# Samaretas/global-motion-estimation

Hardware: AMD Instinct MI355X
Metric: frame-pairs/s + achieved HBM GB/s, 720x480 bs=16 sw=16 exhaustive (higher is better)
Workload: dtype u8; 1 GPU; 720x480 synthetic luma, bs=16 sw=16 exhaustive MAE (BASELINE configs[1]); frame_distance=1, streams_per_gpu=1, collective=none, exchange=none in this run, multi_gpu_measured_by_builder=False

## Files before the change

global-motion-estimation_amd/csrc/bbme_sea.hip:

```cpp
#include "bbme_sea_common.h"

namespace {

using namespace sea;

constexpr int GUARD_NONE = 0, GUARD_ROWS = 1, GUARD_ALL = 2;
constexpr uint32_t PENALTY = 1u << 17;
constexpr uint32_t FIRST_INVALID_KEY = 65536u << 13;
constexpr uint32_t FIRST_INVALID_BOUND = FIRST_INVALID_KEY >> 13;
__device__ __forceinline__ uint32_t lds_add_rtn(uint32_t* p, uint32_t v)
{
    uint32_t old;
    const uint32_t addr = (uint32_t)(uintptr_t)(__attribute__((address_space(3))) uint32_t*)p;
    asm volatile("ds_add_rtn_u32 %0, %1, %2\n\ts_waitcnt lgkmcnt(0)" : "=v"(old) : "v"(addr), "v"(v) : "memory");
    return old;
}
constexpr uint32_t ENT_INTERIOR = 1u << 29;
__device__ __forceinline__ int wave_row(const SeaGeo& d, int w)
{
    if (__builtin_constant_p(d.tc) && (d.tc & (d.tc - 1)) == 0) return w >> __builtin_ctz((unsigned)d.tc);
    return div_small(w, d.magic_tc);
}
__device__ __forceinline__ uint64_t any_u64()
{
// ... 132 lines not shown
            for (int s = 0; s < 4; ++s) w[s] = *(const u64_a4*)(lrow + t * d.pitch_dw + s);
#pragma unroll
            for (int i = 0; i < R; ++i) {
                const int a = t - i;
                if (a < 0 || a > 3) continue;
                const u32x4 ar = *(const u32x4*)(an + a * 4);
#pragma unroll
                for (int j = 0; j < 4; ++j)
                    acc[i] = __builtin_amdgcn_qsad_pk_u16_u8(w[j], ar[j], acc[i]);
            }
        }
    }
#pragma unroll
    for (int i = 0; i < R; ++i) {
        uint32_t lo = (uint32_t)acc[i], hi = (uint32_t)(acc[i] >> 32);
        lo += (uint32_t)__builtin_amdgcn_update_dpp(0, (int)lo, 0xB1, 0xF, 0xF, false);
        hi += (uint32_t)__builtin_amdgcn_update_dpp(0, (int)hi, 0xB1, 0xF, 0xF, false);
        lo += (uint32_t)__builtin_amdgcn_update_dpp(0, (int)lo, 0x4E, 0xF, 0xF, false);
        hi += (uint32_t)__builtin_amdgcn_update_dpp(0, (int)hi, 0x4E, 0xF, 0xF, false);
        asm volatile("" : "+v"(lo), "+v"(hi));
        acc[i] = ((uint64_t)hi << 32) | lo;
    }
    uint32_t key = 0xFFFFFFFFu;
    if (active) {
        const int ci = q2 * 4 * R + 4 * k2 + sub, ri0 = prow2 * R;
        const uint32_t shift = (uint32_t)(sub & 1) * 16u;
        if (ent & ENT_INTERIOR) {
#pragma unroll
            for (int i = 0; i < R; ++i) {
                const uint32_t word = (sub & 2) ? (uint32_t)(acc[i] >> 32) : (uint32_t)acc[i];
                const uint32_t sad = __builtin_amdgcn_ubfe(word, shift, 16u);
                key = min(key, (sad << 13) + (uint32_t)i);
            }
            key += (uint32_t)(ci * NC + ri0);
        } else {
            const int c02 = (bcol0 + wc2) * 16, r02 = (trow * d.tr + wr2) * 16;
            const int lo_c = max(0, d.sw - c02), hi_c = min(NC - 1, W - 16 - c02 + d.sw);
            const int lo_r2 = max(0, d.sw - r02), hi_r2 = min(NC - 1, H - 16 - r02 + d.sw);
#pragma unroll
            for (int i = 0; i < R; ++i) {
                const int ri = ri0 + i;
                if (ci < lo_c || ci > hi_c || ri < lo_r2 || ri > hi_r2) continue;
                const uint32_t word = (sub & 2) ? (uint32_t)(acc[i] >> 32) : (uint32_t)acc[i];
                const uint32_t sad = __builtin_amdgcn_ubfe(word, shift, 16u);
                key = min(key, (sad << 13) | (uint32_t)(ci * NC + ri));
            }
        }
        key = min(key, (uint32_t)__builtin_amdgcn_update_dpp(-1, (int)key, 0xB1, 0xF, 0xF, false));
        key = min(key, (uint32_t)__builtin_amdgcn_update_dpp(-1, (int)key, 0x4E, 0xF, 0xF, false));
    }
    return key;
}

template <int R, bool FIXED, bool VERT>
__device__ __forceinline__ bool tile_phases(const SeaGeo& d, uint32_t* lds, const Layout& L, int pair, int trow, int bcol0,
                                            uint32_t mine, uint32_t pa, uint32_t pb, int tid, int tile_id, PhaseClock& clk)
{
    constexpr bool E4 = R >= 3;
    const int T = blockDim.x;
    const int NC = 2 * d.sw + 16, XQ = d.xq;
    uint32_t* win = lds + L.win;
    uint32_t* anchor = lds + L.anchor;
    uint32_t* best = lds + L.best;
    uint32_t* count = lds + L.count;
    uint64_t* s8 = (uint64_t*)(lds + L.s8);
    uint32_t* work = lds + L.work;
    const int wave = __builtin_amdgcn_readfirstlane(tid >> 6);
    const int lane = tid & 63;
    const SeaArgs c = launch_args();
    const WaveBlock wb = wave_block(d, c, trow, bcol0, wave);
    const int brow = wb.brow, bcol = wb.bcol;
    const bool wave_ok = wb.ok;
    const int r0 = brow * 16, c0 = bcol * 16;
    const int prow = lane >> 2, q = lane & 3;

    box_sums8<R, FIXED>(d, win, s8, tid);
    clk.mark(ST_BOX, lane);
    __syncthreads();
    clk.mark(ST_BOX_WAIT, lane);

    const int lo_r = max(0, d.sw - r0), hi_r = min(NC - 1, c->H - 16 - r0 + d.sw);
    const bool rows_inside = NC == 16 * R && lo_r == 0 && hi_r == NC - 1;
    uint32_t ub_key = 0xFFFFFFFFu;
    if (wave_ok) {
        const int lo_c = max(0, d.sw - c0), hi_c = min(NC - 1, c->W - 16 - c0 + d.sw);
        uint32_t pmin[R];
        const uint64_t* s8blk = s8 + 16 * wb.wr * XQ + wb.wc * 4;
        const uint64_t* sp0 = s8blk + prow * R * XQ + q * R;
        const bool cols_inside = NC == 16 * R && lo_c == 0 && hi_c == NC - 1;
        if (rows_inside && cols_inside)
            lower_bounds<R, GUARD_NONE, VERT>(sp0, XQ, prow, q, pa, pb, lo_r, hi_r, lo_c, hi_c, pmin);
        else if (R <= 3 && cols_inside)
            lower_bounds<R, GUARD_ROWS, VERT>(sp0, XQ, prow, q, pa, pb, lo_r, hi_r, lo_c, hi_c, pmin);
        else
            lower_bounds<R, GUARD_ALL, VERT>(sp0, XQ, prow, q, pa, pb, lo_r, hi_r, lo_c, hi_c, pmin);
        const uint32_t first_idx = (uint32_t)((q * 4 * R) * NC + prow * R);
        const uint32_t ent0 = (rows_inside && cols_inside ? ENT_INTERIOR : 0u) | ((uint32_t)wave << 25) | ((uint32_t)lane << 19);
        uint32_t pkd[R], lane_min = 0xFFFFFFFFu;
#pragma unroll
        for (int k = 0; k < R; ++k) {
            pkd[k] = (pmin[k] << 13) | (first_idx + (uint32_t)(4 * k * NC));
            lane_min = min(lane_min, pmin[k]);
        }
        const uint32_t lane_lb = lane_min << 13;
        uint32_t lb_key = lane_min != 0xFFFFFFFFu ? lane_lb + ((uint32_t)lane << 7) : 0xFFFFFFFFu;
        lb_key = wave_min_u32(lb_key);
        {
            const int idx1 = min_bound_candidate<R, VERT>(s8blk, XQ, NC, (int)(lb_key >> 7) & 63, lb_key >> 13, pa, pb,
                                                          lo_r, hi_r, lo_c, hi_c, lane);
            const int idx0 = d.sw * NC + d.sw;
            const int arow = lane >> 2, aj = lane & 3;
            uint32_t packed = 0;
#pragma unroll
            for (int which = 0; which < 2; ++which) {
                const int idx = which ? idx1 : idx0;
                const int ci = idx / NC, ri = idx - ci * NC;
                const int byte = wb.wc * 16 + ci + 4 * aj;
                const uint32_t* p = win + (16 * wb.wr + ri + arow) * d.pitch_dw + (byte >> 2);
                const uint32_t v = __builtin_amdgcn_alignbyte(p[1], p[0], (uint32_t)byte & 3u);
                packed += __builtin_amdgcn_sad_u8(v, mine, 0u) << (16 * which);
            }
            packed = wave_sum_u32(packed);
            ub_key = min(((packed & 0xFFFFu) << 13) | (uint32_t)idx0, ((packed >> 16) << 13) | (uint32_t)idx1);
            const int idxp = (int)(best[2 * wave + 1] & 0x1FFFu);
            const int cip = idxp / NC, rip = idxp - cip * NC;
            if (idxp != idx0 && idxp != idx1 && cip >= lo_c && cip <= hi_c && rip >= lo_r && rip <= hi_r) {
                const int byte = wb.wc * 16 + cip + 4 * aj;
                const uint32_t* p = win + (16 * wb.wr + rip + arow) * d.pitch_dw + (byte >> 2);
                const uint32_t v = __builtin_amdgcn_alignbyte(p[1], p[0], (uint32_t)byte & 3u);
                const uint32_t sadp = wave_sum_u32(__builtin_amdgcn_sad_u8(v, mine, 0u));
                ub_key = min(ub_key, (sadp << 13) | (uint32_t)idxp);
            }
// ... 200 lines not shown
                        }
                    key += (uint32_t)(ci0 * NC + ri0);
                } else {
                    const int c02 = (bcol0 + wc2) * 16, r02 = (trow * d.tr + wr2) * 16;
                    const int lo_c = max(0, d.sw - c02), hi_c = min(NC - 1, W - 16 - c02 + d.sw);
                    const int lo_r2 = max(0, d.sw - r02), hi_r2 = min(NC - 1, H - 16 - r02 + d.sw);
    #pragma unroll
                    for (int e4 = 0; e4 < 4; ++e4) {
                        const int ci = ci0 + e4;
                        if (ci < lo_c || ci > hi_c) continue;
    #pragma unroll
                        for (int i = 0; i < R; ++i) {
                            const int ri = ri0 + i;
                            if (ri < lo_r2 || ri > hi_r2) continue;
                            const uint32_t sad = (uint32_t)(acc[i] >> (16 * e4)) & 0xFFFFu;
                            key = min(key, (sad << 13) | (uint32_t)(ci * NC + ri));
                        }
                    }
                }
                if (key != 0xFFFFFFFFu) atomicMin(&best[2 * w2], key);
            }
            clk.mark(ST_E, lane);
            __syncthreads();
            clk.mark(ST_E_WAIT, lane);
        }

    }
    if (wave_ok && lane == 0) {
        const int idx = (int)(best[2 * wave] & 0x1FFF);
        const int ci = idx / NC, ri = idx - ci * NC;
        int32_t* o = ce->mf + (((long long)pair * ce->nbr + brow) * ce->nbc + bcol) * 2;
        o[0] = ci - d.sw;
        o[1] = ri - d.sw;
        best[2 * wave + 1] = (uint32_t)idx;
    }
    return false;
}

template <int R, bool FIXED = false, bool VERT = true>
struct MaeTile {
    struct Pre { uint32_t pa, pb; };
    static __device__ __forceinline__ Pre prep(uint32_t* lds, const Layout& L, int wave, int lane, bool wave_ok, uint32_t mine)
    {
        Pre p = { 0, 0 };
        if (wave_ok) {
            lds[L.anchor + wave * ANCHOR_STRIDE + lane] = mine;
            uint32_t a01, a23;
            anchor_quadrants(mine, &a01, &a23);
            p.pa = VERT ? pair_u16(a01, a23, false) : a01;
            p.pb = VERT ? pair_u16(a01, a23, true) : a23;
        }
        return p;
    }
    static __device__ __forceinline__ bool phases(const SeaGeo& d, uint32_t* lds, const Layout& L, int pair, int trow, int bcol0,
                                                  uint32_t mine, const Pre& p, int tid, int tile_id, PhaseClock& clk)
    {
        return tile_phases<R, FIXED, VERT>(d, lds, L, pair, trow, bcol0, mine, p.pa, p.pb, tid, tile_id, clk);
    }
    static __device__ __forceinline__ int probe_word(const Layout& L, int wave) { return L.best + 2 * wave + 1; }
};

template <int R>
__global__ void __launch_bounds__(1024) k_exh_sea16(SeaDev d)
{
    extern __shared__ uint32_t lds[];
    const SeaGeo g = d;
    one_tile<MaeTile<R>>(g, lds, layout_of(g, R));
}

constexpr bool vertical_pairs(int R, int NV) { return !(R == 5 && NV == 16); }

template <int R, int NV, int GEO = 0>
__global__ void __launch_bounds__(1024, (R <= 3 ? 8 : 6)) k_exh_sea16p(SeaDev d)
{
    extern __shared__ uint32_t lds[];
    SeaGeo g = d;
    fix_geometry<R, GEO>(g);
    const Layout L = layout_of(g, R);
    if ((threadIdx.x & 63) == 0) lds[L.best + 2 * (threadIdx.x >> 6) + 1] = (uint32_t)(g.sw * (2 * g.sw + 16) + g.sw);
    persistent_tiles<NV, MaeTile<R, GEO != 0, vertical_pairs(R, NV)>>(g, lds, L);
}

struct MaeLaunch {
    static constexpr const char* persistent_name = "k_exh_sea16p";
    static constexpr const char* one_tile_name = "k_exh_sea16";
    static int no_plan()
    {
        gme_set_error("search window too large for LDS");
        return GME_ERR_ARG;
    }
    static void tables(SeaDev& d, const BbmeJob&) { d.sqbox = nullptr; d.sqbox_stride = 0; }
    static void ordered(SeaDev& d)
    {
        d.quota = getenv("GME_SEA_QUOTA") ? atoi(getenv("GME_SEA_QUOTA")) : SEA_DEFAULT_QUOTA;
        d.bisect = getenv("GME_SEA_BISECT") ? atoi(getenv("GME_SEA_BISECT")) : SEA_DEFAULT_BISECT;
        d.engage = getenv("GME_SEA_ENGAGE") ? atoi(getenv("GME_SEA_ENGAGE")) : SEA_DEFAULT_ENGAGE;
        if (d.engage < d.quota) d.engage = d.quota;
    }
    static bool fits(int R, int nv) { return R <= 1 || R >= 4 || nv <= 8; }
    template <int R, int NV, int GEO = 0>
    static void persistent(dim3 grid, dim3 block, size_t lds, hipStream_t s, const SeaDev& d)
    {
        hipLaunchKernelGGL((k_exh_sea16p<R, NV, GEO>), grid, block, lds, s, d);
    }
    template <int R>
    static void one_tile(dim3 grid, dim3 block, size_t lds, hipStream_t s, const SeaDev& d)
    {
        hipLaunchKernelGGL((k_exh_sea16<R>), grid, block, lds, s, d);
    }
};

}

bool bbme_sea_applies(int bs, int sw, int procedure, int pnorm)
{
    if (procedure != GME_SEARCH_EXHAUSTIVE || bs != 16 || pnorm != GME_NORM_MAE) return false;
    if (sw < 0 || sw % 4 != 0) return false;
    const int NC = 2 * sw + 16;
    return (NC + 15) / 16 <= 5 && NC * NC <= 8192 && !getenv("GME_FORCE_GENERIC") && !getenv("GME_EXH_BRUTE");
}

#ifdef SEA_PHASE_STAMPS
int sea_stamps_read_mse(unsigned long long* out, int reset);
extern "C" GME_API int gme_sea_phase_stamps(int norm, unsigned long long* out, int reset)
{
    return norm ? sea_stamps_read_mse(out, reset) : sea::sea_stamps_read(out, reset);
}
#endif

int launch_bbme_sea(gme_ctx* ctx, const BbmeJob& job, bool* handled)
{
    *handled = false;
    if (!bbme_sea_applies(job.bs, job.sw, job.procedure, job.pnorm)) return GME_OK;
// ... 3 lines not shown
```

global-motion-estimation_amd/csrc/bbme_sea_common.h:

```cpp
#pragma once
#include <stdlib.h>

#include "gme_internal.h"

namespace sea {

constexpr double SHARE_WEIGHT = 0.5;

struct SeaGeo {
    int sw;
    int tr, tc, nb;
    uint32_t magic_tc;
    int pitch_dw, win_rows;
    int s8_rows;
    int rstep;
    uint32_t magic_pitch;
    uint32_t magic_xq;
    int xq;
};

struct SeaDev : SeaGeo {
    unsigned long long magic_wpp;
    unsigned long long magic_wpr;
    const uint8_t* cur;
// ... 21 lines not shown
#pragma clang diagnostic pop

typedef const __attribute__((address_space(4))) SeaDev* SeaArgs;
__device__ __forceinline__ SeaArgs launch_args()
{
    SeaArgs p = (SeaArgs)__builtin_amdgcn_kernarg_segment_ptr();
    asm volatile("" : "+s"(p));
    return p;
}
static_assert(sizeof(SeaDev) % 8 == 0, "the hidden arguments start right behind SeaDev");
__device__ __forceinline__ int launch_groups_x(SeaArgs c)
{
    return (int)*(const __attribute__((address_space(4))) uint32_t*)(c + 1);
}

typedef uint64_t u64_a4 __attribute__((aligned(4)));

enum {
    ST_HEAD,
    ST_HEAD_WAIT,
    ST_FETCH,
    ST_BOX,
    ST_BOX_WAIT,
    ST_BC,
    ST_C2,
    ST_D,
    ST_D_WAIT,
    ST_E,
    ST_E_WAIT,
    ST_F_TAIL,
    ST_TILES,
    ST_SLOTS = 16
};
#ifdef SEA_PHASE_STAMPS
static __device__ unsigned long long stamp_totals[16 * ST_SLOTS];
struct PhaseClock {
    uint32_t slot, last;
    __device__ __forceinline__ void start(uint32_t* totals, int wave)
    {
        slot = (uint32_t)(uintptr_t)(__attribute__((address_space(3))) uint32_t*)(totals + wave * ST_SLOTS);
        last = (uint32_t)__builtin_amdgcn_s_memtime();
    }
    __device__ __forceinline__ void add(int span, int lane, uint32_t v)
    {
        if (lane == 0) asm volatile("ds_add_u32 %0, %1" : : "v"(slot + 4u * (uint32_t)span), "v"(v) : "memory");
    }
    __device__ __forceinline__ void mark(int span, int lane)
    {
        const uint32_t now = (uint32_t)__builtin_amdgcn_s_memtime();
        add(span, lane, now - last);
        last = now;
    }
};
inline int sea_stamps_read(unsigned long long* out, int reset)
{
    GME_HIP_TRY(hipDeviceSynchronize());
    GME_HIP_TRY(hipMemcpyFromSymbol(out, HIP_SYMBOL(stamp_totals), sizeof(stamp_totals)));
    if (reset) {
        void* p = nullptr;
        GME_HIP_TRY(hipGetSymbolAddress(&p, HIP_SYMBOL(stamp_totals)));
        GME_HIP_TRY(hipMemset(p, 0, sizeof(stamp_totals)));
    }
    return GME_OK;
}
#else
struct PhaseClock {
    __device__ __forceinline__ void add(int, int, uint32_t) {}
    __device__ __forceinline__ void mark(int, int) {}
};
#endif


#define SEA_DPP(v, ctrl) GME_DPP(v, ctrl)

constexpr uint32_t div_magic(int dv) { return (1u << 20) / (uint32_t)dv + 1u; }
inline unsigned long long div_magic40(int dv) { return (1ull << 40) / (unsigned long long)dv + 1ull; }
__device__ __forceinline__ int div_small(int n, uint32_t magic) { return (int)(__umul24((uint32_t)n, magic) >> 20); }

__device__ __forceinline__ bool locate(const SeaGeo& d, SeaArgs c, int* pair, int* trow, int* bcol0)
{
    *pair = (int)blockIdx.z * 8 + (int)(blockIdx.x & 7);
    *trow = (int)blockIdx.y;
    *bcol0 = (int)(blockIdx.x >> 3) * d.tc;
    return *pair < c->pairs;
}

inline bool grid_for(const SeaDev& d, dim3* grid)
{
    const long long gz = ((long long)d.pairs + 7) / 8;
    if (gz > 65535 || d.tile_rows > 65535) return false;
    *grid = dim3((unsigned)(8 * d.wg_per_row), (unsigned)d.tile_rows, (unsigned)gz);
    return true;
}

constexpr int ANCHOR_STRIDE = 68;
typedef uint32_t u32x4 __attribute__((ext_vector_type(4)));

struct Layout {
    int win, anchor, best, count, a2, prev, own, s8, work, total;
#ifdef SEA_PHASE_STAMPS
    int stamps;
#endif
};

__host__ __device__ constexpr Layout make_layout(int R, int nb, int win_rows, int pitch_dw, int xq, int s8_rows)
{
    Layout l{};
// ... 13 lines not shown
#endif
    return l;
}

__device__ __forceinline__ Layout layout_of(const SeaGeo& d, int R)
{
    return make_layout(R, d.nb, d.win_rows, d.pitch_dw, d.xq, d.s8_rows);
}

struct WaveBlock {
    int wr, wc;
    int brow, bcol;
    bool ok;
};
__device__ __forceinline__ WaveBlock wave_block(const SeaGeo& d, SeaArgs c, int trow, int bcol0, int wave)
{
    WaveBlock b;
    b.wr = div_small(wave, d.magic_tc);
    b.wc = wave - b.wr * d.tc;
    b.brow = trow * d.tr + b.wr;
    b.bcol = bcol0 + b.wc;
    b.ok = b.bcol < c->nbc && b.brow < c->nbr;
    return b;
}

__device__ __forceinline__ void stage_window(const SeaGeo& d, SeaArgs c, uint32_t* win, const uint8_t* cur, int bcol0, int r0)
{
    const int pitch = c->pitch, H = c->H;
    const int gx0 = bcol0 * 16 - d.sw, gy0 = r0 - d.sw;
    const int rstep = d.rstep;
    const int row0 = div_small((int)threadIdx.x, d.magic_pitch), dw = (int)threadIdx.x - row0 * d.pitch_dw;
    const int gx = gx0 + 4 * dw;
    const bool colok = gx >= 0 && gx < pitch;
    if (row0 < rstep) {
        const uint8_t* src = cur + (long long)(gy0 + row0) * pitch + gx;
        const long long sstep = (long long)rstep * pitch;
        uint32_t* dst = win + threadIdx.x;
        const int dstep = rstep * d.pitch_dw;
        for (int row = row0; row < d.win_rows; row += 4 * rstep, src += 4 * sstep, dst += 4 * dstep) {
            uint32_t v[4];
#pragma unroll
            for (int u = 0; u < 4; ++u) {
                const int gy = gy0 + row + u * rstep;
                v[u] = 0;
                if (colok && row + u * rstep < d.win_rows && gy >= 0 && gy < H) v[u] = *(const uint32_t*)(src + u * sstep);
            }
#pragma unroll
            for (int u = 0; u < 4; ++u)
                if (row + u * rstep < d.win_rows) dst[u * dstep] = v[u];
        }
    }
}

template <int CH, bool FIXED>
__device__ __forceinline__ void box_sums8_ch(const SeaGeo& d, const uint32_t* win, uint64_t* s8, int tid, int need)
{
    static_assert((CH + 7) * 1020 < 65536, "cumulative 4-byte sums must fit 16 bits");
    const int XQ = d.xq;
    const int wave = __builtin_amdgcn_readfirstlane(tid >> 6), lane = tid & 63;
    const int SL = XQ == need ? XQ + 1 : XQ;
    const bool wide = SL > 64;
    const uint32_t magic_sl = XQ == need ? div_magic(SL) : d.magic_xq;
    const int SEG = wide ? 1 : div_small(64, magic_sl);
    const int units = wide ? 8 * div_small(XQ + 62, div_magic(63)) : 8;
    const int ls = wide ? 0 : div_small(lane, magic_sl);
    const int RB = FIXED ? 254 / d.pitch_dw + 1 : 1;
    for (int u = wave * SEG; u < units; u += d.nb * SEG) {
        __builtin_amdgcn_s_setprio(1);
        const int ch = wide ? (u & 7) : u + ls;
        const int sq = wide ? (u >> 3) * 63 + lane : lane - ls * SL;
        const bool active = wide ? sq < SL : (ls < SEG && ch < 8);
        const bool stores = active && sq < XQ && (!wide || lane < 63);
        int pi = active ? (ch * CH) * d.pitch_dw + sq : 0, oi = (ch * CH) * XQ + sq;
        constexpr int ROWS = CH + 7, STEP = FIXED ? 8 : 1, AHEAD = FIXED ? 16 : 1;
        uint64_t ring[8], acc = 0, w[ROWS];
        int read = 0;
#pragma unroll
        for (int r = 0; r < ROWS; ++r) {
            if (r % STEP == 0) {
#pragma unroll
                for (; read < ROWS && read < r + AHEAD; ++read) {
                    if constexpr (FIXED) {
                        if (read > 0 && read % RB == 0) {
                            pi += RB * d.pitch_dw;
                            asm volatile("" : "+v"(pi));
                        }
                        w[read] = *(const u64_a4*)(win + pi + (read % RB) * d.pitch_dw);
                    } else {
                        w[read] = *(const u64_a4*)(win + pi);
                        pi += d.pitch_dw;
                        asm volatile("" : "+v"(pi));
                    }
                }
            }
            acc = __builtin_amdgcn_qsad_pk_u16_u8(w[r], 0u, acc);
            if (r >= 7) {
                uint32_t lo = (uint32_t)acc, hi = (uint32_t)(acc >> 32);
                if (r >= 8) { lo -= (uint32_t)ring[r & 7]; hi -= (uint32_t)(ring[r & 7] >> 32); }
                lo += SEA_DPP(lo, 0x130);
                hi += SEA_DPP(hi, 0x130);
                asm volatile("" : "+v"(lo), "+v"(hi));
                if constexpr (FIXED) {
                    if (stores) s8[oi + (r - 7) * XQ] = ((uint64_t)hi << 32) | lo;
                } else {
                    if (stores) s8[oi] = ((uint64_t)hi << 32) | lo;
                    oi += XQ;
                    asm volatile("" : "+v"(oi));
                }
            }
            ring[r & 7] = acc;
        }
        __builtin_amdgcn_s_setprio(0);
    }
}

template <int R, bool FIXED>
__device__ __forceinline__ void box_sums8(const SeaGeo& d, const uint32_t* win, uint64_t* s8, int tid)
{
    const int need = 4 * R + 4 * (d.tc - 1) + 2;
    if (d.tr == 1) box_sums8_ch<2 * R + 1, FIXED>(d, win, s8, tid, need);
    else if (d.tr == 2) box_sums8_ch<2 * R + 3, FIXED>(d, win, s8, tid, need);
    else box_sums8_ch<2 * R + 7, FIXED>(d, win, s8, tid, need);
}

__device__ __forceinline__ void anchor_quadrants(uint32_t mine, uint32_t* a01, uint32_t* a23)
{
    uint32_t s = __builtin_amdgcn_sad_u8(mine, 0u, 0u);
    s += SEA_DPP(s, 0xB1);
    s += SEA_DPP(s, 0x124);
    s += SEA_DPP(s, 0x128);
    const uint32_t q0 = (uint32_t)__builtin_amdgcn_readlane((int)s, 0) + (uint32_t)__builtin_amdgcn_readlane((int)s, 16);
    const uint32_t q1 = (uint32_t)__builtin_amdgcn_readlane((int)s, 2) + (uint32_t)__builtin_amdgcn_readlane((int)s, 18);
    const uint32_t q2 = (uint32_t)__builtin_amdgcn_readlane((int)s, 32) + (uint32_t)__builtin_amdgcn_readlane((int)s, 48);
    const uint32_t q3 = (uint32_t)__builtin_amdgcn_readlane((int)s, 34) + (uint32_t)__builtin_amdgcn_readlane((int)s, 50);
    *a01 = q0 | (q1 << 16);
    *a23 = q2 | (q3 << 16);
}

constexpr int box_conflicts(int xq, int R)
{
    int worst = 0, hits[64] = {};
    for (int b = 0; b < 64; ++b) hits[b] = 0;
    for (int prow = 0; prow < 8; ++prow)
        for (int q = 0; q < 4; ++q) {
            const int dw = 2 * ((prow * R) * xq + q * R);
            ++hits[dw & 63]; ++hits[(dw + 1) & 63];
        }
    for (int b = 0; b < 64; ++b) worst = hits[b] > worst ? hits[b] : worst;
    return worst;
}
constexpr int pick_xq(int need, int R)
{
    int best = need, best_c = 1 << 30;
    for (int x = need; x < need + 12; ++x) {
        const int c = box_conflicts(x, R);
        if (c < best_c) { best_c = c; best = x; }
    }
    return best;
}

constexpr int pick_pitch(int need, int R)
{
    int best_p = need, best_c = 1 << 30;
    for (int p = need; p < need + 16; ++p) {
        int quad = 0, seen[32] = {};
        for (int i = 0; i < 32; ++i) seen[i] = 0;
        for (int sub = 0; sub < 4; ++sub) { quad += seen[(4 * sub * p) & 31]; ++seen[(4 * sub * p) & 31]; quad += seen[(4 * sub * p + 1) & 31]; }
        int probe = 0;
        for (int i = 0; i < 32; ++i) seen[i] = 0;
        for (int row = 0; row < 8; ++row)
            for (int dw = 0; dw < 4; ++dw) probe += seen[(row * p + dw) & 31]++;
        const int c = 64 * quad + probe + 2 * (p - need);
        if (c < best_c) { best_c = c; best_p = p; }
    }
    (void)R;
// ... 87 lines not shown
constexpr double REDO_DEFAULT_FRAC = 0.75;

__device__ __forceinline__ void push_redo(SeaArgs c, int tile_in_xcd, int xcd)
{
    uint32_t* status = c->status;
    const uint32_t slot = atomicAdd(status + GME_STATUS_REDO, 1u);
    c->redo_list[slot] = ((uint32_t)tile_in_xcd << 3) | (uint32_t)xcd;
    atomicAdd(status + GME_STATUS_STATS + 16 * xcd + 1, 1u);
}

template <class Below>
__device__ __forceinline__ uint32_t first_round_limit(SeaArgs c, uint32_t lo, uint32_t hi, int shift, Below below)
{
    const int bisect = c->bisect, quota = c->quota;
    if (bisect < 0) return (lo + ((hi - lo) >> -bisect) + 1) << shift;
    for (int s = 0; s < bisect && lo < hi; ++s) {
        const uint32_t mid = (lo + hi) >> 1;
        if ((int)below((mid + 1) << shift) > quota) hi = mid; else lo = mid;
    }
    return (lo + 1) << shift;
}

__device__ __forceinline__ int tile_number(const SeaGeo& d, SeaArgs c, int pair, int trow, int bcol0)
{
    return (pair >> 3) * c->wg_per_pair + trow * c->wg_per_row + div_small(bcol0, d.magic_tc);
}


template <class Kern>
__device__ __forceinline__ void one_tile(const SeaGeo& d, uint32_t* lds, const Layout L)
{
    const SeaArgs c = launch_args();
    int pair, trow, bcol0;
    if (!locate(d, c, &pair, &trow, &bcol0)) return;
    const int wave = __builtin_amdgcn_readfirstlane(threadIdx.x >> 6);
    const int lane = threadIdx.x & 63;
    const long long plane = (long long)pair * c->plane_stride;
    stage_window(d, c, lds + L.win, c->cur + plane, bcol0, trow * d.tr * 16);
    uint32_t mine = 0;
    const WaveBlock wb = wave_block(d, c, trow, bcol0, wave);
    if (wb.ok) {
        const int pitch = c->pitch;
        const uint8_t* aptr = c->prev + plane + (long long)(wb.brow * 16) * pitch + wb.bcol * 16;
        mine = *(const uint32_t*)(aptr + (uint32_t)((lane >> 2) * pitch + (lane & 3) * 4));
    }
    const typename Kern::Pre pre = Kern::prep(lds, L, wave, lane, wb.ok, mine);
    if (lane == 0) lds[Kern::probe_word(L, wave)] = (uint32_t)(d.sw * (2 * d.sw + 16) + d.sw);
    if (threadIdx.x == 0) { lds[L.count] = 0; lds[L.count + 4] = 0; lds[L.count + 5] = 0; lds[L.count + 7] = 0; }
    __syncthreads();
    PhaseClock clk;
#ifdef SEA_PHASE_STAMPS
    clk.start(lds + L.stamps, wave);
#endif
    Kern::phases(d, lds, L, pair, trow, bcol0, mine, pre, (int)threadIdx.x, tile_number(d, c, pair, trow, bcol0), clk);
    if (threadIdx.x == 0) {
        uint32_t* stats = launch_args()->status + GME_STATUS_STATS + 16 * (blockIdx.x & 7);
        atomicAdd(stats, lds[L.count] + lds[L.count + 5]);
        atomicAdd(stats + 2, lds[L.count] + lds[L.count + 4]);
    }
}

__device__ __forceinline__ int tiles_of_xcd(SeaArgs c, int xcd) { return ((c->pairs - xcd + 7) >> 3) * c->wg_per_pair; }
__device__ __forceinline__ uint32_t* tile_counter(SeaArgs c, int xcd) { return c->dynamic ? c->status + GME_STATUS_TILECTR + 16 * xcd : nullptr; }

template <int NV, class Kern>
__device__ __forceinline__ void persistent_tiles(const SeaGeo& d, uint32_t* lds, const Layout L)
{
    const int xcd = blockIdx.x & 7;
    int tile = blockIdx.x >> 3;
    if (tile >= tiles_of_xcd(launch_args(), xcd)) return;
    int tid_carried = (int)threadIdx.x;
    auto opaque_tid = [&]() {
        asm volatile("" : "+v"(tid_carried));
        return tid_carried;
    };

    uint32_t wv[NV], an_next = 0;
    int pair = 0, trow = 0, bcol0 = 0;
    auto fetch = [&](int t, int tid) {
        const SeaArgs c = launch_args();
        const int wave = __builtin_amdgcn_readfirstlane(tid >> 6), lane = tid & 63;
        const int row0 = div_small(tid, d.magic_pitch), dw = tid - row0 * d.pitch_dw;
        const int lp = (int)(((unsigned long long)(unsigned)t * c->magic_wpp) >> 40);
        const int wg = t - lp * c->wg_per_pair;
        const int wpr = c->wg_per_row;
        trow = (int)(((unsigned long long)(unsigned)wg * c->magic_wpr) >> 40);
        bcol0 = (wg - trow * wpr) * d.tc;
        pair = lp * 8 + xcd;
        const int pitch = c->pitch;
        const long long plane = (long long)pair * c->plane_stride;
        const uint8_t* cur = c->cur + plane;
        const unsigned long long cur_bits = (unsigned long long)cur;
        const __amdgpu_buffer_rsrc_t rs = __builtin_amdgcn_make_buffer_rsrc(
            (void*)(((unsigned long long)(unsigned)__builtin_amdgcn_readfirstlane((int)(cur_bits >> 32)) << 32) |
                    (unsigned)__builtin_amdgcn_readfirstlane((int)cur_bits)),
            (short)0, __builtin_amdgcn_readfirstlane(c->H * pitch), 0x00020000);
        const int gx0 = bcol0 * 16 - d.sw + 4 * dw, gy0 = trow * d.tr * 16 - d.sw + row0;
        const bool colok = row0 < d.rstep && gx0 >= 0 && gx0 < pitch;
        int outside = (int)0x80000000;
        asm volatile("" : "+v"(outside));
        const int off0 = colok ? gy0 * pitch + gx0 : outside;
        const int sstep = d.rstep * pitch;
#pragma unroll
        for (int u = 0; u < NV; ++u)
            wv[u] = (uint32_t)__builtin_amdgcn_raw_buffer_load_b32(rs, off0 + u * sstep, 0, 0);
        an_next = 0;
        const WaveBlock wb = wave_block(d, c, trow, bcol0, wave);
        if (wb.ok) {
            const uint8_t* aptr = c->prev + plane + (long long)(wb.brow * 16) * pitch + wb.bcol * 16;
            an_next = *(const uint32_t*)(aptr + (uint32_t)((lane >> 2) * pitch + (lane & 3) * 4));
        }
    };
    fetch(tile, opaque_tid());
    uint32_t drawn = 0;
    if (opaque_tid() == 0) {
        if (uint32_t* ctr = tile_counter(launch_args(), xcd)) drawn = atomicInc(ctr, 0xFFFFFFFFu);
        lds[L.count] = 0; lds[L.count + 3] = 0; lds[L.count + 4] = 0; lds[L.count + 5] = 0; lds[L.count + 7] = 0;
    }
    uint32_t stat_scored = 0, stat_listed = 0;
    PhaseClock clk;
#ifdef SEA_PHASE_STAMPS
    {
        const int tid = opaque_tid();
        if (tid < d.nb * ST_SLOTS) lds[L.stamps + tid] = 0;
        __syncthreads();
        clk.start(lds + L.stamps, __builtin_amdgcn_readfirstlane(tid >> 6));
    }
#endif
    for (;;) {
        const int tid = opaque_tid();
        const int wave = __builtin_amdgcn_readfirstlane(tid >> 6), lane = tid & 63;
        const int gx = launch_groups_x(launch_args()) >> 3;
        {
            const int row0 = div_small(tid, d.magic_pitch);
            if (row0 < d.rstep) {
                uint32_t* dst = lds + L.win + tid;
                const int dstep = d.rstep * d.pitch_dw;
#pragma unroll
                for (int u = 0; u < NV; ++u)
                    if (row0 + u * d.rstep < d.win_rows) dst[u * dstep] = wv[u];
            }
        }
        const int pair_c = pair, trow_c = trow, bcol0_c = bcol0, tile_c = tile;
        const uint32_t mine = an_next;
        const typename Kern::Pre pre = Kern::prep(lds, L, wave, lane, wave_block(d, launch_args(), trow_c, bcol0_c, wave).ok, mine);
        if (tid == 0) {
            const uint32_t listed = lds[L.count], c2_off = lds[L.count + 4], c2_scored = lds[L.count + 5];
            stat_scored += listed + c2_scored;
            stat_listed += listed + c2_off;
            lds[L.count] = 0; lds[L.count + 4] = 0; lds[L.count + 5] = 0; lds[L.count + 7] = 0;
            lds[L.count + 1] = (uint32_t)gx + drawn;
        }
        clk.mark(ST_HEAD, lane);
        __syncthreads();
        clk.mark(ST_HEAD_WAIT, lane);
        bool more, dynamic;
        {
            const SeaArgs c = launch_args();
            dynamic = c->dynamic != 0;
            tile = dynamic ? (int)lds[L.count + 1] : tile + (launch_groups_x(c) >> 3);
            more = tile < tiles_of_xcd(c, xcd);
            if (more) {
                fetch(tile, tid);
                if (dynamic && tid == 0) drawn = atomicInc(c->status + GME_STATUS_TILECTR + 16 * xcd, 0xFFFFFFFFu);
            }
        }
        clk.mark(ST_FETCH, lane);
        if (!Kern::phases(d, lds, L, pair_c, trow_c, bcol0_c, mine, pre, tid, tile_c, clk)) {
            if (tid == 0) lds[L.count + 3] = 0;
        } else if (dynamic && wave == 0) {
            const int streak = (int)lds[L.count + 3];
            const int burst = streak == 0 ? 0 : streak == 1 ? 3 : streak == 2 ? 7 : REDO_BURST;
            if (burst) {
                const SeaArgs c = launch_args();
                uint32_t got = 0;
                if (lane >= 1 && lane <= burst) got = atomicAdd(c->status + GME_STATUS_TILECTR + 16 * xcd, 1u);
                const int t = (launch_groups_x(c) >> 3) + (int)(lane == 0 ? drawn : got);
                if (lane < burst && t < tiles_of_xcd(c, xcd)) push_redo(c, t, xcd);
                drawn = (uint32_t)__builtin_amdgcn_readlane((int)got, __builtin_amdgcn_readfirstlane(burst));
            }
            if (lane == 0) lds[L.count + 3] = (uint32_t)(streak + 1);
        }
        clk.mark(ST_F_TAIL, lane);
        clk.add(ST_TILES, lane, 1u);
        if (!more) break;
    }
#ifdef SEA_PHASE_STAMPS
    {
        asm volatile("s_waitcnt lgkmcnt(0)" : : : "memory");
        __syncthreads();
        const int tid = opaque_tid();
        if (tid < d.nb * ST_SLOTS) atomicAdd(stamp_totals + tid, (unsigned long long)lds[L.stamps + tid]);
    }
#endif
    if (opaque_tid() == 0) {
        uint32_t* stats = launch_args()->status + GME_STATUS_STATS + 16 * xcd;
        atomicAdd(stats, stat_scored + lds[L.count] + lds[L.count + 5]);
        atomicAdd(stats + 2, stat_listed + lds[L.count] + lds[L.count + 4]);
    }
}

struct PersistPlan { bool use; bool dynamic; long long g; int nv; };
inline PersistPlan plan_persistent(const SeaDev& d, size_t lds_bytes, int pairs, int cu_count)
{
    PersistPlan p;
    const long long tiles_x = (((long long)pairs + 7) / 8) * d.wg_per_pair;
    p.nv = (d.win_rows + d.rstep - 1) / d.rstep;
    const char* pmode = getenv("GME_SEA_PERSIST");
    const int pm = pmode ? atoi(pmode) : -1;
    int per_cu = (int)((160 * 1024) / (lds_bytes + 1024));
    if (per_cu * d.nb > 32) per_cu = 32 / d.nb;
    if (per_cu < 1) per_cu = 1;
    p.g = (long long)per_cu * cu_count / 8;
    const bool can = tiles_x < (1ll << 21) && d.wg_per_pair < (1 << 18) && p.nv <= 16 && p.g >= 1;
    p.use = can && (pm > 0 || (pm < 0 && tiles_x >= 4 * p.g));
    p.dynamic = pm != 1;
    if (p.g > tiles_x) p.g = tiles_x;
    return p;
}

template <class Norm, int R>
// ... 71 lines not shown
```

global-motion-estimation_amd/csrc/bbme_sea_mse.hip:

```cpp
#include "bbme_sea_common.h"

namespace {

using namespace sea;

typedef short s16x2 __attribute__((ext_vector_type(2)));

__device__ __forceinline__ unsigned long long u64min_(unsigned long long a, unsigned long long b) { return a < b ? a : b; }


__device__ __forceinline__ uint32_t pk_mad_i16(uint32_t a, uint32_t b, uint32_t c)
{
    uint32_t d;
    asm("v_pk_mad_i16 %0, %1, %2, %3" : "=v"(d) : "v"(a), "s"(b), "v"(c));
    return d;
}

template <int R, bool GUARD>
__device__ __forceinline__ void lower_bounds_mse(const uint64_t* sp0, int XQ, int prow, int q, uint32_t a01, uint32_t a23,
                                                 int lo_r, int hi_r, int lo_c, int hi_c, uint32_t (&pkey)[R])
{
#pragma unroll
    for (int k = 0; k < R; ++k) pkey[k] = 0xFFFFFFFFu;
    const uint64_t* top = sp0;
// ... 33 lines not shown
                                                int lo_r, int hi_r, int lo_c, int hi_c, uint32_t (&pkey)[R])
{
#pragma unroll
    for (int k = 0; k < R; ++k) pkey[k] = 0xFFFFFFFFu;
    const uint64_t* top = sp0;
    const uint64_t* bot = sp0 + 8 * XQ;
#pragma unroll
    for (int i = 0; i < R; ++i) {
        const int ri = prow * R + i;
        if (!GUARD || (ri >= lo_r && ri <= hi_r)) {
            uint64_t t[R + 2], b[R + 2];
#pragma unroll
            for (int k = 0; k < R + 2; ++k) { t[k] = top[k]; b[k] = bot[k]; }
#pragma unroll
            for (int k = 0; k < R; ++k) {
                const int ci0 = q * 4 * R + 4 * k;
                if (GUARD && (ci0 > hi_c || ci0 + 3 < lo_c)) continue;
#pragma unroll
                for (int e = 0; e < 4; ++e) {
                    if (GUARD && (ci0 + e < lo_c || ci0 + e > hi_c)) continue;
                    const uint32_t sel = (e & 1) ? 0x07060302u : 0x05040100u;
                    const uint32_t tp = __builtin_amdgcn_perm((uint32_t)(t[k + 2] >> (32 * (e >> 1))), (uint32_t)(t[k] >> (32 * (e >> 1))), sel);
                    const uint32_t bt = __builtin_amdgcn_perm((uint32_t)(b[k + 2] >> (32 * (e >> 1))), (uint32_t)(b[k] >> (32 * (e >> 1))), sel);
                    const uint32_t lb = __builtin_amdgcn_sad_u16(tp, a01, __builtin_amdgcn_sad_u16(bt, a23, 0u));
                    pkey[k] = min(pkey[k], (lb << 13) + (uint32_t)((4 * k + e) * R + i));
                }
            }
        }
        top += XQ;
        bot += XQ;
    }
}

template <int R>
__device__ __forceinline__ uint32_t bounds2_patch(const uint64_t* sp, int XQ, int k, uint32_t a01m, uint32_t a23m)
{
    uint32_t best = 0xFFFFFFFFu;
#pragma unroll
    for (int i = 0; i < R; ++i) {
        const uint64_t t0 = sp[i * XQ + k], t2 = sp[i * XQ + k + 2], b0 = sp[(i + 8) * XQ + k], b2 = sp[(i + 8) * XQ + k + 2];
#pragma unroll
        for (int e = 0; e < 4; ++e) {
            const uint32_t sel = (e & 1) ? 0x07060302u : 0x05040100u;
            const uint32_t tp = __builtin_amdgcn_perm((uint32_t)(t2 >> (32 * (e >> 1))), (uint32_t)(t0 >> (32 * (e >> 1))), sel);
            const uint32_t bt = __builtin_amdgcn_perm((uint32_t)(b2 >> (32 * (e >> 1))), (uint32_t)(b0 >> (32 * (e >> 1))), sel);
            const s16x2 dt = __builtin_bit_cast(s16x2, pk_mad_i16(tp, 0x00020002u, a01m));
            const s16x2 db = __builtin_bit_cast(s16x2, pk_mad_i16(bt, 0x00020002u, a23m));
            best = min(best, (uint32_t)__builtin_amdgcn_sdot2(dt, dt, __builtin_amdgcn_sdot2(db, db, 0, true), true));
        }
    }
    return best >> 7;
}

template <int R, bool FIXED>
__device__ __forceinline__ bool tile_phases_mse(const SeaGeo& d, uint32_t* lds, const Layout& L, int pair, int trow, int bcol0,
                                                uint32_t mine, uint32_t a01, uint32_t a23, uint32_t mine2, int tid, int tile_id, PhaseClock& clk)
{
    constexpr bool TWO = R >= TWO_LEVEL_FROM;
    const int T = blockDim.x;
    const int NC = 2 * d.sw + 16, XQ = d.xq;
    uint32_t* win = lds + L.win;
    uint32_t* anchor = lds + L.anchor;
    unsigned long long* best = (unsigned long long*)(lds + L.best);
    uint32_t* count = lds + L.count;
    uint32_t* a2s = lds + L.a2;
    uint64_t* s8 = (uint64_t*)(lds + L.s8);
    uint32_t* work = lds + L.work;
    const int wave = __builtin_amdgcn_readfirstlane(tid >> 6);
    const int lane = tid & 63;
    const SeaArgs c = launch_args();
    const WaveBlock wb = wave_block(d, c, trow, bcol0, wave);
    const int brow = wb.brow, bcol = wb.bcol;
    const bool wave_ok = wb.ok;
    const int r0 = brow * 16, c0 = bcol * 16;
    const int prow = lane >> 2, q = lane & 3;

    box_sums8<R, FIXED>(d, win, s8, tid);
    clk.mark(ST_BOX, lane);
    __syncthreads();
    clk.mark(ST_BOX_WAIT, lane);

    const int lo_r = max(0, d.sw - r0), hi_r = min(NC - 1, c->H - 16 - r0 + d.sw);
    const bool rows_inside = NC == 16 * R && lo_r == 0 && hi_r == NC - 1;
    if (wave_ok) {
        const int lo_c = max(0, d.sw - c0), hi_c = min(NC - 1, c->W - 16 - c0 + d.sw);
        uint32_t pkey[R];
        const uint64_t* sp0 = s8 + (16 * wb.wr + prow * R) * XQ + wb.wc * 4 + q * R;
        uint32_t patch_lb[R], lb_key = 0xFFFFFFFFu;
        if constexpr (TWO) {
            const uint32_t p01 = __builtin_bit_cast(uint32_t, (s16x2)(-__builtin_bit_cast(s16x2, a01))) >> 1 & 0x7FFF7FFFu;
            const uint32_t p23 = __builtin_bit_cast(uint32_t, (s16x2)(-__builtin_bit_cast(s16x2, a23))) >> 1 & 0x7FFF7FFFu;
            if (rows_inside && lo_c == 0 && hi_c == NC - 1)
                lower_bounds_l1<R, false>(sp0, XQ, prow, q, p01, p23, lo_r, hi_r, lo_c, hi_c, pkey);
            else
                lower_bounds_l1<R, true>(sp0, XQ, prow, q, p01, p23, lo_r, hi_r, lo_c, hi_c, pkey);
            if (lane == 0) { lds[L.own + 2 * wave] = a01; lds[L.own + 2 * wave + 1] = a23; }
#pragma unroll
            for (int k = 0; k < R; ++k) {
                patch_lb[k] = pkey[k] == 0xFFFFFFFFu ? 0xFFFFFFFFu : pkey[k] >> 13;
                lb_key = min(lb_key, pkey[k] == 0xFFFFFFFFu ? 0xFFFFFFFFu : ((pkey[k] >> 13) << 7) | (pkey[k] & 127u));
            }
        } else {
            if (rows_inside && lo_c == 0 && hi_c == NC - 1)
                lower_bounds_mse<R, false>(sp0, XQ, prow, q, a01, a23, lo_r, hi_r, lo_c, hi_c, pkey);
            else
                lower_bounds_mse<R, true>(sp0, XQ, prow, q, a01, a23, lo_r, hi_r, lo_c, hi_c, pkey);
#pragma unroll
            for (int k = 0; k < R; ++k) {
                patch_lb[k] = pkey[k] == 0xFFFFFFFFu ? 0xFFFFFFFFu : pkey[k] >> 7;
                lb_key = min(lb_key, pkey[k]);
            }
        }
        const uint32_t lb_min = wave_min_u32(lb_key);
        unsigned long long ub_key = ~0ull;
        {
            const int bl = __builtin_amdgcn_readfirstlane(__ffsll((long long)__ballot(lb_key == lb_min)) - 1), loc = lb_min & 127;
            const int ce = loc / R, li = loc - ce * R;
            const int idx1 = ((bl & 3) * 4 * R + ce) * NC + (bl >> 2) * R + li;
            const int idx0 = d.sw * NC + d.sw;
            const int arow = lane >> 2, aj = lane & 3;
#pragma unroll
            for (int which = 0; which < 2; ++which) {
                const int idx = which ? idx1 : idx0;
                const int ci = idx / NC, ri = idx - ci * NC;
                const int byte = wb.wc * 16 + ci + 4 * aj;
                const uint32_t* p = win + (16 * wb.wr + ri + arow) * d.pitch_dw + (byte >> 2);
                const uint32_t v = __builtin_amdgcn_alignbyte(p[1], p[0], (uint32_t)byte & 3u);
                const uint32_t part = mine2 + __builtin_amdgcn_udot4(v, v, 0u, false) - 2u * __builtin_amdgcn_udot4(v, mine, 0u, false);
                const uint32_t ssd = wave_sum_u32(part);
                ub_key = u64min_(ub_key, ((unsigned long long)ssd << 13) | (unsigned)idx);
            }
            const int idxp = (int)(lds[L.prev + wave] & 0x1FFFu);
            const int cip = idxp / NC, rip = idxp - cip * NC;
// ... 141 lines not shown
                    for (int i = 0; i < R; ++i) {
                        const uint32_t cost = a2 + b2[i][e4] - 2u * acc[i][e4];
                        key = u64min_(key, ((unsigned long long)cost << 13) | (unsigned)((ci0 + e4) * NC + ri0 + i));
                    }
            } else {
#pragma unroll
                for (int e4 = 0; e4 < 4; ++e4) {
                    const int ci = ci0 + e4;
                    if (ci < lo_c || ci > hi_c) continue;
#pragma unroll
                    for (int i = 0; i < R; ++i) {
                        const int ri = ri0 + i;
                        if (ri < lo_r2 || ri > hi_r2) continue;
                        const uint32_t cost = a2 + sq1(tab, tabrow + (long long)i * pitch + e4) - 2u * acc[i][e4];
                        key = u64min_(key, ((unsigned long long)cost << 13) | (unsigned)(ci * NC + ri));
                    }
                }
            }
            if (key != ~0ull) atomicMin(&best[w2], key);
        }
        clk.mark(ST_E, lane);
        __syncthreads();
        clk.mark(ST_E_WAIT, lane);
    }

    if (wave_ok && lane == 0) {
        const int idx = (int)(best[wave] & 0x1FFF);
        const int ci = idx / NC, ri = idx - ci * NC;
        int32_t* o = ce->mf + (((long long)pair * ce->nbr + brow) * ce->nbc + bcol) * 2;
        o[0] = ci - d.sw;
        o[1] = ri - d.sw;
        lds[L.prev + wave] = (uint32_t)idx;
    }
    return false;
}

template <int R, bool FIXED = false>
struct MseTile {
    struct Pre { uint32_t a01, a23, mine2; };
    static __device__ __forceinline__ Pre prep(uint32_t* lds, const Layout& L, int wave, int lane, bool wave_ok, uint32_t mine)
    {
        Pre p = { 0, 0, 0 };
        if (wave_ok) {
            lds[L.anchor + wave * ANCHOR_STRIDE + lane] = mine;
            anchor_quadrants(mine, &p.a01, &p.a23);
            p.a01 = __builtin_bit_cast(uint32_t, -(__builtin_bit_cast(s16x2, p.a01 << 1)));
            p.a23 = __builtin_bit_cast(uint32_t, -(__builtin_bit_cast(s16x2, p.a23 << 1)));
            p.mine2 = __builtin_amdgcn_udot4(mine, mine, 0u, false);
            const uint32_t a2 = wave_sum_u32(p.mine2);
            if (lane == 0) lds[L.a2 + wave] = a2;
        }
        return p;
    }
    static __device__ __forceinline__ bool phases(const SeaGeo& d, uint32_t* lds, const Layout& L, int pair, int trow, int bcol0,
                                                  uint32_t mine, const Pre& p, int tid, int tile_id, PhaseClock& clk)
    {
        return tile_phases_mse<R, FIXED>(d, lds, L, pair, trow, bcol0, mine, p.a01, p.a23, p.mine2, tid, tile_id, clk);
    }
    static __device__ __forceinline__ int probe_word(const Layout& L, int wave) { return L.prev + wave; }
};

template <int R>
__global__ void __launch_bounds__(1024) k_exh_sea16_mse(SeaDev d)
{
    extern __shared__ uint32_t lds[];
    const SeaGeo g = d;
    one_tile<MseTile<R>>(g, lds, layout_of(g, R));
}

template <int R, int NV, int GEO = 0>
__global__ void __launch_bounds__(1024, (R <= 3 ? 8 : 6)) k_exh_sea16p_mse(SeaDev d)
{
    extern __shared__ uint32_t lds[];
    SeaGeo g = d;
    fix_geometry<R, GEO>(g);
    const Layout L = layout_of(g, R);
    if ((threadIdx.x & 63) == 0) lds[L.prev + (threadIdx.x >> 6)] = (uint32_t)(g.sw * (2 * g.sw + 16) + g.sw);
    persistent_tiles<NV, MseTile<R, GEO != 0>>(g, lds, L);
}

struct MseLaunch {
    static constexpr const char* persistent_name = "k_exh_sea16p_mse";
    static constexpr const char* one_tile_name = "k_exh_sea16_mse";
    static int no_plan() { return GME_OK; }
    static void tables(SeaDev& d, const BbmeJob& job) { d.sqbox = job.sqbox_cur; d.sqbox_stride = job.sqbox_stride; }
    static void ordered(SeaDev& d) { d.quota = 0; d.bisect = 0; d.engage = 0; }
    static bool fits(int R, int nv) { return R != 3 || nv <= 12; }
    template <int R, int NV, int GEO = 0>
    static void persistent(dim3 grid, dim3 block, size_t lds, hipStream_t s, const SeaDev& d)
    {
        hipLaunchKernelGGL((k_exh_sea16p_mse<R, NV, GEO>), grid, block, lds, s, d);
    }
    template <int R>
    static void one_tile(dim3 grid, dim3 block, size_t lds, hipStream_t s, const SeaDev& d)
    {
        hipLaunchKernelGGL((k_exh_sea16_mse<R>), grid, block, lds, s, d);
    }
};

}

#ifdef SEA_PHASE_STAMPS
int sea_stamps_read_mse(unsigned long long* out, int reset) { return sea::sea_stamps_read(out, reset); }
#endif

int launch_bbme_sea_mse(gme_ctx* ctx, const BbmeJob& job, bool* handled)
{
    *handled = false;
    if (job.procedure != GME_SEARCH_EXHAUSTIVE || job.bs != 16 || job.pnorm != GME_NORM_MSE) return GME_OK;
    if (job.sqbox_cur == nullptr || job.sqbox_kind != 1 || job.sw < 0 || job.sw % 4 != 0) return GME_OK;
    if (getenv("GME_FORCE_GENERIC") || getenv("GME_EXH_BRUTE")) return GME_OK;
    const int NC = 2 * job.sw + 16, R = (NC + 15) / 16;
    if (R < 1 || R > 5 || NC * NC > 8192) return GME_OK;
    return launch_sea<MseLaunch>(ctx, job, handled);
}
```

Before: 643,400 frame-pairs/s.

## Defer next-tile prefetch until after box sums for waves owning box chunks

In the persistent tile loop, waves that are assigned box-sum chunks now issue the next tile's global fetch (and dynamic tile-counter atomic) only after the box-sum barrier, via a callback injected into the phase function. Other waves still prefetch immediately. The aim is to keep box-sum waves off the critical path before the barrier while still overlapping the next tile's loads with the search phases. It is enabled per template configuration, with some R/NV/GEO combinations excluded, and it adds a per-wave branch plus a template parameter through the tile-phase functions.

New measurement: 656,100 frame-pairs/s, median of 6. 1.02x the previous value.

```diff
diff --git a/global-motion-estimation_amd/csrc/bbme_sea.hip b/global-motion-estimation_amd/csrc/bbme_sea.hip
--- a/global-motion-estimation_amd/csrc/bbme_sea.hip
+++ b/global-motion-estimation_amd/csrc/bbme_sea.hip
@@ -208,9 +208,10 @@
     return key;
 }
 
-template <int R, bool FIXED, bool VERT>
+template <int R, bool FIXED, bool VERT, class Behind>
 __device__ __forceinline__ bool tile_phases(const SeaGeo& d, uint32_t* lds, const Layout& L, int pair, int trow, int bcol0,
-                                            uint32_t mine, uint32_t pa, uint32_t pb, int tid, int tile_id, PhaseClock& clk)
+                                            uint32_t mine, uint32_t pa, uint32_t pb, int tid, int tile_id, PhaseClock& clk,
+                                            Behind&& behind_box_sums)
 {
     constexpr bool E4 = R >= 3;
     const int T = blockDim.x;
@@ -234,6 +235,7 @@
     clk.mark(ST_BOX, lane);
     __syncthreads();
     clk.mark(ST_BOX_WAIT, lane);
+    behind_box_sums();
 
     const int lo_r = max(0, d.sw - r0), hi_r = min(NC - 1, c->H - 16 - r0 + d.sw);
     const bool rows_inside = NC == 16 * R && lo_r == 0 && hi_r == NC - 1;
@@ -540,11 +542,13 @@
         }
         return p;
     }
+    template <class Behind>
     static __device__ __forceinline__ bool phases(const SeaGeo& d, uint32_t* lds, const Layout& L, int pair, int trow, int bcol0,
-                                                  uint32_t mine, const Pre& p, int tid, int tile_id, PhaseClock& clk)
+                                                  uint32_t mine, const Pre& p, int tid, int tile_id, PhaseClock& clk, Behind&& behind_box_sums)
     {
-        return tile_phases<R, FIXED, VERT>(d, lds, L, pair, trow, bcol0, mine, p.pa, p.pb, tid, tile_id, clk);
-    }
+        return tile_phases<R, FIXED, VERT>(d, lds, L, pair, trow, bcol0, mine, p.pa, p.pb, tid, tile_id, clk, behind_box_sums);
+    }
+    static __device__ __forceinline__ bool holds_chunks(const SeaGeo& d, int wave) { return holds_box_chunks<R>(d, wave); }
     static __device__ __forceinline__ int probe_word(const Layout& L, int wave) { return L.best + 2 * wave + 1; }
 };
 
@@ -557,6 +561,8 @@
 }
 
 constexpr bool vertical_pairs(int R, int NV) { return !(R == 5 && NV == 16); }
+
+constexpr bool late_prefetch(int R, int GEO) { return !(R == 3 && GEO == 0); }
 
 template <int R, int NV, int GEO = 0>
 __global__ void __launch_bounds__(1024, (R <= 3 ? 8 : 6)) k_exh_sea16p(SeaDev d)
@@ -566,7 +572,7 @@
     fix_geometry<R, GEO>(g);
     const Layout L = layout_of(g, R);
     if ((threadIdx.x & 63) == 0) lds[L.best + 2 * (threadIdx.x >> 6) + 1] = (uint32_t)(g.sw * (2 * g.sw + 16) + g.sw);
-    persistent_tiles<NV, MaeTile<R, GEO != 0, vertical_pairs(R, NV)>>(g, lds, L);
+    persistent_tiles<NV, MaeTile<R, GEO != 0, vertical_pairs(R, NV)>, late_prefetch(R, GEO)>(g, lds, L);
 }
 
 struct MaeLaunch {
diff --git a/global-motion-estimation_amd/csrc/bbme_sea_common.h b/global-motion-estimation_amd/csrc/bbme_sea_common.h
--- a/global-motion-estimation_amd/csrc/bbme_sea_common.h
+++ b/global-motion-estimation_amd/csrc/bbme_sea_common.h
@@ -97,7 +97,7 @@
         last = now;
     }
 };
-inline int sea_stamps_read(unsigned long long* out, int reset)
+static inline int sea_stamps_read(unsigned long long* out, int reset)
 {
     GME_HIP_TRY(hipDeviceSynchronize());
     GME_HIP_TRY(hipMemcpyFromSymbol(out, HIP_SYMBOL(stamp_totals), sizeof(stamp_totals)));
@@ -217,17 +217,35 @@
     }
 }
 
+struct BoxDeal {
+    int SL;
+    bool wide;
+    uint32_t magic_sl;
+    int SEG;
+    int units;
+};
+__device__ __forceinline__ BoxDeal box_deal(const SeaGeo& d, int need)
+{
+    BoxDeal b;
+    const int XQ = d.xq;
+    b.SL = XQ == need ? XQ + 1 : XQ;
+    b.wide = b.SL > 64;
+    b.magic_sl = XQ == need ? div_magic(b.SL) : d.magic_xq;
+    b.SEG = b.wide ? 1 : div_small(64, b.magic_sl);
+    b.units = b.wide ? 8 * div_small(XQ + 62, div_magic(63)) : 8;
+    return b;
+}
+
 template <int CH, bool FIXED>
 __device__ __forceinline__ void box_sums8_ch(const SeaGeo& d, const uint32_t* win, uint64_t* s8, int tid, int need)
 {
     static_assert((CH + 7) * 1020 < 65536, "cumulative 4-byte sums must fit 16 bits");
     const int XQ = d.xq;
     const int wave = __builtin_amdgcn_readfirstlane(tid >> 6), lane = tid & 63;
-    const int SL = XQ == need ? XQ + 1 : XQ;
-    const bool wide = SL > 64;
-    const uint32_t magic_sl = XQ == need ? div_magic(SL) : d.magic_xq;
-    const int SEG = wide ? 1 : div_small(64, magic_sl);
-    const int units = wide ? 8 * div_small(XQ + 62, div_magic(63)) : 8;
+    const BoxDeal deal = box_deal(d, need);
+    const int SL = deal.SL, SEG = deal.SEG, units = deal.units;
+    const bool wide = deal.wide;
+    const uint32_t magic_sl = deal.magic_sl;
     const int ls = wide ? 0 : div_small(lane, magic_sl);
     const int RB = FIXED ? 254 / d.pitch_dw + 1 : 1;
     for (int u = wave * SEG; u < units; u += d.nb * SEG) {
@@ -279,13 +297,22 @@
     }
 }
 
+template <int R>
+__device__ __forceinline__ int box_quads_needed(const SeaGeo& d) { return 4 * R + 4 * (d.tc - 1) + 2; }
 template <int R, bool FIXED>
 __device__ __forceinline__ void box_sums8(const SeaGeo& d, const uint32_t* win, uint64_t* s8, int tid)
 {
-    const int need = 4 * R + 4 * (d.tc - 1) + 2;
+    const int need = box_quads_needed<R>(d);
     if (d.tr == 1) box_sums8_ch<2 * R + 1, FIXED>(d, win, s8, tid, need);
     else if (d.tr == 2) box_sums8_ch<2 * R + 3, FIXED>(d, win, s8, tid, need);
     else box_sums8_ch<2 * R + 7, FIXED>(d, win, s8, tid, need);
+}
+
+template <int R>
+__device__ __forceinline__ bool holds_box_chunks(const SeaGeo& d, int wave)
+{
+    const BoxDeal deal = box_deal(d, box_quads_needed<R>(d));
+    return wave * deal.SEG < deal.units;
 }
 
 __device__ __forceinline__ void anchor_quadrants(uint32_t mine, uint32_t* a01, uint32_t* a23)
@@ -479,7 +506,7 @@
 #ifdef SEA_PHASE_STAMPS
     clk.start(lds + L.stamps, wave);
 #endif
-    Kern::phases(d, lds, L, pair, trow, bcol0, mine, pre, (int)threadIdx.x, tile_number(d, c, pair, trow, bcol0), clk);
+    Kern::phases(d, lds, L, pair, trow, bcol0, mine, pre, (int)threadIdx.x, tile_number(d, c, pair, trow, bcol0), clk, [] {});
     if (threadIdx.x == 0) {
         uint32_t* stats = launch_args()->status + GME_STATUS_STATS + 16 * (blockIdx.x & 7);
         atomicAdd(stats, lds[L.count] + lds[L.count + 5]);
@@ -490,7 +517,21 @@
 __device__ __forceinline__ int tiles_of_xcd(SeaArgs c, int xcd) { return ((c->pairs - xcd + 7) >> 3) * c->wg_per_pair; }
 __device__ __forceinline__ uint32_t* tile_counter(SeaArgs c, int xcd) { return c->dynamic ? c->status + GME_STATUS_TILECTR + 16 * xcd : nullptr; }
 
-template <int NV, class Kern>
+template <class Fetch>
+__device__ __forceinline__ void next_tile_of(const uint32_t* lds, const Layout& L, int xcd, int tid, int& tile, bool& more, bool& dynamic,
+                                             uint32_t& drawn, Fetch& fetch)
+{
+    const SeaArgs c = launch_args();
+    dynamic = c->dynamic != 0;
+    tile = dynamic ? (int)lds[L.count + 1] : tile + (launch_groups_x(c) >> 3);
+    more = tile < tiles_of_xcd(c, xcd);
+    if (more) {
+        fetch(tile, tid);
+        if (dynamic && tid == 0) drawn = atomicInc(c->status + GME_STATUS_TILECTR + 16 * xcd, 0xFFFFFFFFu);
+    }
+}
+
+template <int NV, class Kern, bool LATE = true>
 __device__ __forceinline__ void persistent_tiles(const SeaGeo& d, uint32_t* lds, const Layout L)
 {
     const int xcd = blockIdx.x & 7;
@@ -581,19 +622,22 @@
         clk.mark(ST_HEAD, lane);
         __syncthreads();
         clk.mark(ST_HEAD_WAIT, lane);
-        bool more, dynamic;
-        {
-            const SeaArgs c = launch_args();
-            dynamic = c->dynamic != 0;
-            tile = dynamic ? (int)lds[L.count + 1] : tile + (launch_groups_x(c) >> 3);
-            more = tile < tiles_of_xcd(c, xcd);
-            if (more) {
-                fetch(tile, tid);
-                if (dynamic && tid == 0) drawn = atomicInc(c->status + GME_STATUS_TILECTR + 16 * xcd, 0xFFFFFFFFu);
+        bool more = false, dynamic = false;
+        bool holds = false;
+        if constexpr (LATE) holds = Kern::holds_chunks(d, wave);
+        if (!holds) {
+            next_tile_of(lds, L, xcd, tid, tile, more, dynamic, drawn, fetch);
+            clk.mark(ST_FETCH, lane);
+        }
+        auto behind_box_sums = [&]() __attribute__((always_inline)) {
+            if constexpr (LATE) {
+                if (holds) {
+                    next_tile_of(lds, L, xcd, tid, tile, more, dynamic, drawn, fetch);
+                    clk.mark(ST_FETCH, lane);
+                }
             }
-        }
-        clk.mark(ST_FETCH, lane);
-        if (!Kern::phases(d, lds, L, pair_c, trow_c, bcol0_c, mine, pre, tid, tile_c, clk)) {
+        };
+        if (!Kern::phases(d, lds, L, pair_c, trow_c, bcol0_c, mine, pre, tid, tile_c, clk, behind_box_sums)) {
             if (tid == 0) lds[L.count + 3] = 0;
         } else if (dynamic && wave == 0) {
             const int streak = (int)lds[L.count + 3];
diff --git a/global-motion-estimation_amd/csrc/bbme_sea_mse.hip b/global-motion-estimation_amd/csrc/bbme_sea_mse.hip
--- a/global-motion-estimation_amd/csrc/bbme_sea_mse.hip
+++ b/global-motion-estimation_amd/csrc/bbme_sea_mse.hip
@@ -109,9 +109,10 @@
     return best >> 7;
 }
 
-template <int R, bool FIXED>
+template <int R, bool FIXED, class Behind>
 __device__ __forceinline__ bool tile_phases_mse(const SeaGeo& d, uint32_t* lds, const Layout& L, int pair, int trow, int bcol0,
-                                                uint32_t mine, uint32_t a01, uint32_t a23, uint32_t mine2, int tid, int tile_id, PhaseClock& clk)
+                                                uint32_t mine, uint32_t a01, uint32_t a23, uint32_t mine2, int tid, int tile_id, PhaseClock& clk,
+                                                Behind&& behind_box_sums)
 {
     constexpr bool TWO = R >= TWO_LEVEL_FROM;
     const int T = blockDim.x;
@@ -136,6 +137,7 @@
     clk.mark(ST_BOX, lane);
     __syncthreads();
     clk.mark(ST_BOX_WAIT, lane);
+    behind_box_sums();
 
     const int lo_r = max(0, d.sw - r0), hi_r = min(NC - 1, c->H - 16 - r0 + d.sw);
     const bool rows_inside = NC == 16 * R && lo_r == 0 && hi_r == NC - 1;
@@ -383,11 +385,13 @@
         }
         return p;
     }
+    template <class Behind>
     static __device__ __forceinline__ bool phases(const SeaGeo& d, uint32_t* lds, const Layout& L, int pair, int trow, int bcol0,
-                                                  uint32_t mine, const Pre& p, int tid, int tile_id, PhaseClock& clk)
+                                                  uint32_t mine, const Pre& p, int tid, int tile_id, PhaseClock& clk, Behind&& behind_box_sums)
     {
-        return tile_phases_mse<R, FIXED>(d, lds, L, pair, trow, bcol0, mine, p.a01, p.a23, p.mine2, tid, tile_id, clk);
-    }
+        return tile_phases_mse<R, FIXED>(d, lds, L, pair, trow, bcol0, mine, p.a01, p.a23, p.mine2, tid, tile_id, clk, behind_box_sums);
+    }
+    static __device__ __forceinline__ bool holds_chunks(const SeaGeo& d, int wave) { return holds_box_chunks<R>(d, wave); }
     static __device__ __forceinline__ int probe_word(const Layout& L, int wave) { return L.prev + wave; }
 };
 
@@ -398,6 +402,8 @@
     const SeaGeo g = d;
     one_tile<MseTile<R>>(g, lds, layout_of(g, R));
 }
+
+constexpr bool late_prefetch_mse(int R, int NV, int GEO) { return !(GEO == 0 && (((R == 3 || R == 5) && NV == 16) || (R == 4 && NV == 12))); }
 
 template <int R, int NV, int GEO = 0>
 __global__ void __launch_bounds__(1024, (R <= 3 ? 8 : 6)) k_exh_sea16p_mse(SeaDev d)
@@ -407,7 +413,7 @@
     fix_geometry<R, GEO>(g);
     const Layout L = layout_of(g, R);
     if ((threadIdx.x & 63) == 0) lds[L.prev + (threadIdx.x >> 6)] = (uint32_t)(g.sw * (2 * g.sw + 16) + g.sw);
-    persistent_tiles<NV, MseTile<R, GEO != 0>>(g, lds, L);
+    persistent_tiles<NV, MseTile<R, GEO != 0>, late_prefetch_mse(R, NV, GEO)>(g, lds, L);
 }
 
 struct MseLaunch {
```
